# snap-research/GiGL

Hardware: AMD Instinct MI355X
Metric: sampled+aggregated edges/s (higher is better)
Workload: dtype f32

## Files before the change

### gigl_amd/csrc/union.hip

```cpp
#include "common.h"

#include <mutex>

#include <cstdlib>

static hipError_t lds_opt_in(int device, int site, const void* fn, int bytes, const void* fn2 = nullptr, int bytes2 = 0) {
  static std::mutex mu;
  static uint32_t done[256] = {0};
  std::lock_guard<std::mutex> lk(mu);
  const uint32_t bit = 1u << site;
  uint32_t& d = done[device & 255];
  if (d & bit) return hipSuccess;
  hipError_t e = hipFuncSetAttribute(fn, hipFuncAttributeMaxDynamicSharedMemorySize, bytes);
  if (e == hipSuccess && fn2) e = hipFuncSetAttribute(fn2, hipFuncAttributeMaxDynamicSharedMemorySize, bytes2);
  if (e == hipSuccess) d |= bit;
  return e;
}

static bool lg_big_cap_wide() {
  static const bool wide = [] {
    const char* e = getenv("GIGL_LG_BIG_CAP");
    return !(e && atoi(e) > 0 && atoi(e) <= 4096);
  }();
  return wide;
// ... 1508 lines not shown
    hipLaunchKernelGGL(lg2_insert_kernel, grid(T_in), dim3(TB), 0, st, a, g);
    hipLaunchKernelGGL(lg2_extras_kernel, grid(S0), dim3(TB), 0, st, a, g);
  }
  {
    gigl_prof_scope ps(ctx, GIGL_K_UNION_NODES);
    hipLaunchKernelGGL(lg2_count_kernel, dim3((unsigned)n_tiles), dim3(256), 0, st, a, g, tile_counts, n_tiles,
                       ticket_count);
    hipLaunchKernelGGL(lg2_assign_kernel, dim3((unsigned)n_tiles), dim3(256), 0, st, a, g, tile_counts, n_tiles,
                       out->nodes, out->meta, out->rowptr, out->rowend, cursor, edge_counters + 32, sort_rows,
                       sort_count, tiny_rows, tiny_count);
  }
  {
    gigl_prof_scope ps(ctx, GIGL_K_UNION_EDGE_SORT);
    hipLaunchKernelGGL(lg2_fill_kernel, grid(T_in), dim3(TB), 0, st, a, g, out->rowend, out->col, out->root_local,
                       out->rowptr);
  }
  {
    gigl_prof_scope ps(ctx, GIGL_K_UNION_CSR);
    {
      int64_t tb = (T_in / 16 + 255) / 256;
      if (tb > 1024) tb = 1024;
      if (tb < 16) tb = 16;
      hipLaunchKernelGGL(lg2_row_sort_tiny_kernel, dim3((unsigned)tb), dim3(256), 0, st, tiny_rows, tiny_count,
                         out->rowptr, out->rowend, out->col, edge_counters);
    }
    int64_t blocks = (T_in / 8 + 3) / 4;
    if (blocks > 256 * 16) blocks = 256 * 16;
    if (blocks < 64) blocks = 64;
    hipLaunchKernelGGL(lg2_row_sort_kernel, dim3((unsigned)blocks), dim3(256), 0, st, sort_rows, sort_count,
                       out->rowptr, out->rowend, out->col, big_rows, big_count, edge_counters);
    if (lg_big_cap_wide()) {
      GIGL_HIP_CHECK(ctx, lds_opt_in(ctx->device, 0, (const void*)lg2_row_sort_big_kernel<BIG_ROW_CAP>, 2 * BIG_ROW_CAP * (int)sizeof(int32_t)));
      hipLaunchKernelGGL(lg2_row_sort_big_kernel<BIG_ROW_CAP>, dim3(8), dim3(1024), 2 * BIG_ROW_CAP * sizeof(int32_t), st,
                       out->rowptr, out->rowend, out->col, big_rows, big_count, out->meta + GIGL_META_OVERFLOW,
                       edge_counters, ticket_big, out->meta);
    } else
    hipLaunchKernelGGL(lg2_row_sort_big_kernel<LG_BIG_CAP>, dim3(8), dim3(1024), 2 * LG_BIG_CAP * sizeof(int32_t), st,
                       out->rowptr, out->rowend, out->col, big_rows, big_count, out->meta + GIGL_META_OVERFLOW,
                       edge_counters, ticket_big, out->meta);
  }
  GIGL_HIP_CHECK(ctx, hipGetLastError());
  return GIGL_OK;
}


constexpr int LG3_CODE_BITS = 20;
constexpr uint32_t LG3_CODE_MASK = (1u << LG3_CODE_BITS) - 1u;
constexpr uint32_t LG3_EMPTY = 0xFFFFFFFFu;
constexpr int32_t LG3_XTAG = 1 << 30;
constexpr int LG3_MAX_PARTS = 16;
constexpr int LG3_NT_DEFAULT = 512;
constexpr int LG3_CAP_DEFAULT = 16384;

struct Lg3Args {
  const uint32_t* roots;
  const uint32_t* nbr0;
  const uint32_t* nbr1;
  const int32_t* cnt0;
  const int32_t* cnt1;
  int32_t b, f0, f1;
  int64_t S0;
  int32_t gr;
  int32_t S0g;
  int32_t Tg;
  int32_t n_groups;
  int32_t P;
  uint32_t cmask;
  uint32_t rmask;
  int32_t rs_shift;
  int32_t bl_shift;
  int32_t* fpw;
  int32_t* fpx;
  int32_t* lid_in;
  int32_t* rowcnt;
  int32_t alias_base;
  int32_t whole_rows;
  int32_t* overflow;
};

__device__ __forceinline__ uint32_t lg3_part(uint32_t h32, int P) { return (uint32_t)(((uint64_t)h32 * (uint32_t)P) >> 32); }

__device__ __forceinline__ int64_t lg3_gpos(const Lg3Args& a, int32_t grp, uint32_t code) {
  return code < (uint32_t)a.gr ? (int64_t)grp * a.gr + code : (int64_t)a.b + (int64_t)grp * a.S0g + (code - a.gr);
}

__device__ __forceinline__ void lg3_locate(const Lg3Args& a, int64_t t, int32_t& grp, uint32_t& code) {
  if (t < a.b) {
    grp = a.n_groups == 1 ? 0 : (int32_t)((uint32_t)t / (uint32_t)a.gr);
    code = (uint32_t)(t - (int64_t)grp * a.gr);
  } else {
    const uint32_t p = (uint32_t)(t - a.b);
    grp = a.n_groups == 1 ? 0 : (int32_t)(p / (uint32_t)a.S0g);
    code = (uint32_t)a.gr + (p - (uint32_t)grp * (uint32_t)a.S0g);
  }
}

__device__ __forceinline__ bool lg3_insert(unsigned long long* table, const Lg3Args& a, uint32_t id, uint32_t h32,
                                           uint32_t code) {
  const unsigned long long mine1 = ((unsigned long long)id << 32) | ((unsigned long long)code << 1) | 1ull;
  uint32_t s = h32 & a.cmask;
  for (uint32_t probes = 0; probes <= a.cmask; ++probes) {
    unsigned long long w = table[s];
    if (w == ~0ull) {
      w = atomicCAS(&table[s], ~0ull, mine1);
      if (w == ~0ull) return true;
    }
    if ((uint32_t)(w >> 32) == id) {
      atomicMin(&table[s], mine1 & ~1ull);
      atomicAnd(&table[s], ~1ull);
      return true;
    }
    s = (s + 1) & a.cmask;
  }
  return false;
}

__device__ __forceinline__ uint32_t lg3_lookup(const unsigned long long* table, const Lg3Args& a, uint32_t id,
                                               uint32_t h32) {
  uint32_t s = h32 & a.cmask;
  for (uint32_t probes = 0; probes <= a.cmask; ++probes) {
    const unsigned long long w = table[s];
    if (w == ~0ull) return LG3_EMPTY;
    if ((uint32_t)(w >> 32) == id) return (uint32_t)w;
    s = (s + 1) & a.cmask;
  }
  return LG3_EMPTY;
}

__device__ __forceinline__ bool lg3_rset_has(const uint32_t* rset, const Lg3Args& a, uint32_t id, uint32_t h32) {
  uint32_t s = (h32 * 0x9E3779B1u) >> a.rs_shift;
  for (;;) {
    const uint32_t k = rset[s];
    if (k == id) return true;
    if (k == GIGL_INVALID) return false;
    s = (s + 1) & a.rmask;
  }
}

__device__ __forceinline__ bool lg3_contributes(const Lg3Args& a, uint32_t first_code, uint32_t my_code, int c) {
  if (c >= a.f1 || !a.whole_rows) return true;
  return first_code == my_code || first_code < (uint32_t)a.gr;
}

__device__ __forceinline__ bool lg3_row_is_segment(const Lg3Args& a, uint32_t code, int c) {
  return a.alias_base >= 0 && a.whole_rows && c < a.f1 && code >= (uint32_t)a.gr;
}

constexpr int LG3_TC = 5;

template <int NT>
__global__ __launch_bounds__(NT) void lg3_dedup_kernel(Lg3Args a, int32_t* tile_counts, int32_t n_tiles,
                                                         int32_t* ticket, int32_t* sort_count, int32_t* tiny_count) {
  extern __shared__ unsigned long long lg3_lds[];
  unsigned long long* table = lg3_lds;
  uint32_t* rset = reinterpret_cast<uint32_t*>(table + (a.cmask + 1u));
  uint32_t* bloom = rset + (a.rmask + 1u);
  int32_t* tcnt = reinterpret_cast<int32_t*>(bloom + ((a.rmask + 1u) >> 2));
  __shared__ int32_t s_last;
  __shared__ int32_t s_w[NT / 64][LG3_TC];
  const int tid = threadIdx.x, lane = tid & 63, wv = tid >> 6;
  uint32_t vid = blockIdx.x;
  if ((gridDim.x & 7u) == 0) vid = (blockIdx.x >> 3) + (blockIdx.x & 7u) * (gridDim.x >> 3);
  const int32_t grp = (int32_t)(vid / (uint32_t)a.P);
  const int q = (int)(vid % (uint32_t)a.P);
  const int64_t r0 = (int64_t)grp * a.gr, p0 = (int64_t)grp * a.S0g;
  const int32_t tile_lo_r = (int32_t)(r0 >> 10), nt_r = (int32_t)((r0 + a.gr - 1) >> 10) - tile_lo_r + 1;
  const int32_t tile_lo_h = (int32_t)((a.b + p0) >> 10), nt_h = (int32_t)((a.b + p0 + a.S0g - 1) >> 10) - tile_lo_h + 1;
  for (uint32_t i = tid; i <= a.cmask; i += NT) table[i] = ~0ull;
  for (uint32_t i = tid; i <= a.rmask; i += NT) rset[i] = GIGL_INVALID;
  for (uint32_t i = tid; i < ((a.rmask + 1u) >> 2); i += NT) bloom[i] = 0u;
  for (int i = tid; i < LG3_TC * (nt_r + nt_h); i += NT) tcnt[i] = 0;
  __syncthreads();
  int32_t over = 0;
  for (int32_t tl = tid; tl < a.gr; tl += NT) {
    const uint32_t id = a.roots[r0 + tl];
    if (id == GIGL_INVALID) continue;
    const uint32_t h = hash_u32(id);
    uint32_t s = (h * 0x9E3779B1u) >> a.rs_shift;
    for (;;) {
      const uint32_t prev = atomicCAS(&rset[s], GIGL_INVALID, id);
      if (prev == GIGL_INVALID || prev == id) break;
      s = (s + 1) & a.rmask;
    }
    const uint32_t bi = (h * 0x85EBCA6Bu) >> a.bl_shift;
    atomicOr(&bloom[bi >> 5], 1u << (bi & 31));
    if ((int)lg3_part(h, a.P) == q && !lg3_insert(table, a, id, h, (uint32_t)tl)) ++over;
  }
  __syncthreads();
  constexpr int PF = 8;
  unsigned long long rootmask = 0;
  for (int32_t base = 0, it0 = 0; base < a.S0g; base += PF * NT, it0 += PF) {
    uint32_t ids[PF], hh[PF], sl[PF], bw[PF];
    uint32_t pend = 0, valid = 0;
#pragma unroll
    for (int u = 0; u < PF; ++u) {
      const int32_t pl = base + u * NT + tid;
      ids[u] = pl < a.S0g ? a.nbr0[p0 + pl] : GIGL_INVALID;
    }
#pragma unroll
    for (int u = 0; u < PF; ++u) {
      hh[u] = hash_u32(ids[u]);
      sl[u] = hh[u] & a.cmask;
      const uint32_t bi = (hh[u] * 0x85EBCA6Bu) >> a.bl_shift;
      bw[u] = (bloom[bi >> 5] >> (bi & 31)) & 1u;
      if (ids[u] != GIGL_INVALID) {
        valid |= 1u << u;
        if ((int)lg3_part(hh[u], a.P) == q) pend |= 1u << u;
      }
    }
    for (uint32_t rounds = 0; pend; ++rounds) {
      if (rounds > a.cmask) {
        over += __popc(pend);
        break;
      }
      unsigned long long old[PF];
#pragma unroll
      for (int u = 0; u < PF; ++u)
        if (pend >> u & 1u)
          old[u] = atomicCAS(&table[sl[u]], ~0ull,
                             ((unsigned long long)ids[u] << 32) | ((unsigned long long)(uint32_t)(a.gr + base + u * NT + tid) << 1) | 1ull);
#pragma unroll
      for (int u = 0; u < PF; ++u) {
        if (!(pend >> u & 1u)) continue;
        if (old[u] == ~0ull) {
          pend &= ~(1u << u);
        } else if ((uint32_t)(old[u] >> 32) == ids[u]) {
          atomicMin(&table[sl[u]], ((unsigned long long)ids[u] << 32) | ((unsigned long long)(uint32_t)(a.gr + base + u * NT + tid) << 1));
          atomicAnd(&table[sl[u]], ~1ull);
          pend &= ~(1u << u);
        } else {
          sl[u] = (sl[u] + 1) & a.cmask;
        }
      }
    }
#pragma unroll
    for (int u = 0; u < PF; ++u) {
      if (!((valid >> u & 1u) && bw[u])) continue;
      if (!lg3_rset_has(rset, a, ids[u], hh[u])) continue;
      rootmask |= 1ull << (it0 + u);
      const int32_t pl = base + u * NT + tid;
      const int c = a.cnt1[p0 + pl];
      const uint32_t* kids = a.nbr1 + (p0 + pl) * a.f1;
      for (int j = 0; j < c; ++j) {
        const uint32_t cid = kids[j];
        const uint32_t ch = hash_u32(cid);
        if ((int)lg3_part(ch, a.P) == q && !lg3_insert(table, a, cid, ch, (uint32_t)(a.Tg + pl * a.f1 + j))) ++over;
      }
    }
  }
  if (over) atomicAdd(a.overflow, over);
  __syncthreads();
  for (int32_t tl = tid; tl < a.gr; tl += NT) {
    const uint32_t id = a.roots[r0 + tl];
    if (id == GIGL_INVALID) {
      if (q == 0) a.fpw[r0 + tl] = -1;
      continue;
    }
    const uint32_t h = hash_u32(id);
    if ((int)lg3_part(h, a.P) != q) continue;
    const uint32_t w = lg3_lookup(table, a, id, h);
    if (w == LG3_EMPTY) {
      a.fpw[r0 + tl] = -1;
      continue;
    }
    const uint32_t code = (w >> 1) & LG3_CODE_MASK;
    a.fpw[r0 + tl] = (int32_t)(code | ((w & 1u) ? 0u : 0x80000000u));
    if (code == (uint32_t)tl) atomicAdd(&tcnt[LG3_TC * (int)(((r0 + tl) >> 10) - tile_lo_r) + 0], 1);
    const int c0 = a.cnt0[r0 + tl];
    if (c0 > 0) atomicAdd(&a.rowcnt[r0 + code], c0);
  }
  for (int32_t base = 0, it0 = 0; base < a.S0g; base += PF * NT, it0 += PF) {
    uint32_t ids[PF], sl[PF], lw[PF];
    int32_t cc[PF];
    uint32_t pend = 0;
#pragma unroll
    for (int u = 0; u < PF; ++u) {
      const int32_t pl = base + u * NT + tid;
      ids[u] = pl < a.S0g ? a.nbr0[p0 + pl] : GIGL_INVALID;
      cc[u] = pl < a.S0g ? a.cnt1[p0 + pl] : 0;
    }
#pragma unroll
    for (int u = 0; u < PF; ++u) {
      const uint32_t h = hash_u32(ids[u]);
      sl[u] = h & a.cmask;
      lw[u] = LG3_EMPTY;
      if (ids[u] != GIGL_INVALID && (int)lg3_part(h, a.P) == q) pend |= 1u << u;
    }
    const uint32_t mine = pend;
    for (uint32_t rounds = 0; pend && rounds <= a.cmask; ++rounds) {
      unsigned long long wv8[PF];
#pragma unroll
      for (int u = 0; u < PF; ++u)
        if (pend >> u & 1u) wv8[u] = table[sl[u]];
#pragma unroll
      for (int u = 0; u < PF; ++u) {
        if (!(pend >> u & 1u)) continue;
        if (wv8[u] == ~0ull) {
          pend &= ~(1u << u);
        } else if ((uint32_t)(wv8[u] >> 32) == ids[u]) {
          lw[u] = (uint32_t)wv8[u];
          pend &= ~(1u << u);
        } else {
          sl[u] = (sl[u] + 1) & a.cmask;
        }
      }
    }
#pragma unroll
    for (int u = 0; u < PF; ++u) {
      const int32_t pl = base + u * NT + tid;
      const uint32_t id = ids[u];
      const int c = cc[u];
      const bool in = pl < a.S0g;
      const int32_t my_tile = (int32_t)((a.b + p0 + pl) >> 10) - tile_lo_h;
      bool first = false;
      if (in && id == GIGL_INVALID) {
        if (q == 0) a.fpw[a.b + p0 + pl] = -1;
      } else if (in && (mine >> u & 1u)) {
        const uint32_t mycode = (uint32_t)(a.gr + pl);
        const uint32_t w = lw[u];
        if (w == LG3_EMPTY) {
          a.fpw[a.b + p0 + pl] = -1;
        } else {
          const uint32_t code = (w >> 1) & LG3_CODE_MASK;
          const bool multi = !(w & 1u);
          a.fpw[a.b + p0 + pl] = (int32_t)(code | (multi ? 0x80000000u : 0u));
          first = code == mycode;
          if ((multi || a.alias_base < 0) && c > 0 && !lg3_row_is_segment(a, code, c) && lg3_contributes(a, code, mycode, c))
            atomicAdd(&a.rowcnt[lg3_gpos(a, grp, code)], c);
        }
      }
      {
        const int32_t tile0 = __builtin_amdgcn_readfirstlane(my_tile);
        const unsigned long long f0m = __ballot(first && my_tile == tile0), f1m = __ballot(first && my_tile != tile0);
        if (lane == 0) {
          if (f0m) atomicAdd(&tcnt[LG3_TC * (nt_r + tile0) + 1], (int32_t)__popcll(f0m));
          if (f1m) atomicAdd(&tcnt[LG3_TC * (nt_r + tile0 + 1) + 1], (int32_t)__popcll(f1m));
        }
      }
      if (rootmask >> (it0 + u) & 1ull) {
        const uint32_t* kids = a.nbr1 + (p0 + pl) * a.f1;
        for (int j = 0; j < c; ++j) {
          const uint32_t cid = kids[j];
          const uint32_t ch = hash_u32(cid);
          if ((int)lg3_part(ch, a.P) != q) continue;
          const uint32_t xcode = (uint32_t)(a.Tg + pl * a.f1 + j);
          const uint32_t w = lg3_lookup(table, a, cid, ch);
          int32_t out = -1;
          if (w != LG3_EMPTY) {
            const uint32_t code = (w >> 1) & LG3_CODE_MASK;
            out = (int32_t)(code | ((w & 1u) ? 0u : 0x80000000u));
            if (code == xcode) atomicAdd(&tcnt[LG3_TC * (nt_r + my_tile) + 1], 1);
          }
          a.fpx[(p0 + pl) * a.f1 + j] = out;
        }
      }
    }
  }
  __syncthreads();
  for (int32_t tl = tid; tl < a.gr; tl += NT) {
    const uint32_t id = a.roots[r0 + tl];
    if (id == GIGL_INVALID || (int)lg3_part(hash_u32(id), a.P) != q) continue;
    const int32_t w = a.fpw[r0 + tl];
    if (w == -1 || ((uint32_t)w & 0x7FFFFFFFu) != (uint32_t)tl) continue;
    const int32_t len = __hip_atomic_load(&a.rowcnt[r0 + tl], __ATOMIC_RELAXED, __HIP_MEMORY_SCOPE_AGENT);
    int32_t* tc = &tcnt[LG3_TC * (int)(((r0 + tl) >> 10) - tile_lo_r)];
    if (len) atomicAdd(&tc[2], len);
    if (len >= 2 && w < 0) atomicAdd(&tc[len > TINY_ROW ? 3 : 4], 1);
  }
  for (int32_t base = 0; base < a.S0g; base += PF * NT) {
    uint32_t ids[PF];
    int32_t cc[PF], ww[PF], len[PF];
#pragma unroll
    for (int u = 0; u < PF; ++u) {
      const int32_t pl = base + u * NT + tid;
      ids[u] = pl < a.S0g ? a.nbr0[p0 + pl] : GIGL_INVALID;
      cc[u] = pl < a.S0g ? a.cnt1[p0 + pl] : 0;
      ww[u] = pl < a.S0g ? a.fpw[a.b + p0 + pl] : -1;
    }
#pragma unroll
    for (int u = 0; u < PF; ++u) {
      const int32_t pl = base + u * NT + tid;
      len[u] = -1;
      if (ids[u] == GIGL_INVALID || ww[u] == -1 || (int)lg3_part(hash_u32(ids[u]), a.P) != q) continue;
      const uint32_t mycode = (uint32_t)(a.gr + pl);
      if (((uint32_t)ww[u] & 0x7FFFFFFFu) != mycode) continue;
      const bool multi = ww[u] < 0;
      if (a.alias_base >= 0 && (!multi || lg3_row_is_segment(a, mycode, cc[u]))) continue;
      len[u] = __hip_atomic_load(&a.rowcnt[a.b + p0 + pl], __ATOMIC_RELAXED, __HIP_MEMORY_SCOPE_AGENT);
    }
#pragma unroll
    for (int u = 0; u < PF; ++u) {
      const int32_t pl = base + u * NT + tid;
      const int32_t my_tile = (int32_t)((a.b + p0 + pl) >> 10) - tile_lo_h;
      const int32_t tile0 = __builtin_amdgcn_readfirstlane(my_tile);
      const bool have = len[u] > 0, sorted = len[u] >= 2 && ww[u] < 0;
      if (!__ballot(have)) continue;
      const bool t0 = my_tile == tile0;
      const unsigned long long q0 = __ballot(sorted && len[u] > TINY_ROW && t0), q1 = __ballot(sorted && len[u] > TINY_ROW && !t0);
      const unsigned long long s0 = __ballot(sorted && len[u] <= TINY_ROW && t0), s1 = __ballot(sorted && len[u] <= TINY_ROW && !t0);
      const int32_t n0 = __builtin_amdgcn_readlane(gigl_wave_incl_scan(have && t0 ? len[u] : 0), 63);
      const int32_t n1 = __builtin_amdgcn_readlane(gigl_wave_incl_scan(have && !t0 ? len[u] : 0), 63);
      if (lane == 0) {
        int32_t* tc = &tcnt[LG3_TC * (nt_r + tile0)];
        if (n0) atomicAdd(&tc[2], n0);
        if (q0) atomicAdd(&tc[3], (int32_t)__popcll(q0));
        if (s0) atomicAdd(&tc[4], (int32_t)__popcll(s0));
        if (n1) atomicAdd(&tc[LG3_TC + 2], n1);
        if (q1) atomicAdd(&tc[LG3_TC + 3], (int32_t)__popcll(q1));
        if (s1) atomicAdd(&tc[LG3_TC + 4], (int32_t)__popcll(s1));
      }
    }
  }
  __syncthreads();
  for (int i = tid; i < LG3_TC * (nt_r + nt_h); i += NT) {
    const int32_t v = tcnt[i];
    if (v) {
      const int k = i / LG3_TC;
      const int32_t tile = k < nt_r ? tile_lo_r + k : tile_lo_h + (k - nt_r);
      atomicAdd(&tile_counts[tile * LG3_TC + (i - k * LG3_TC)], v);
    }
  }
  __syncthreads();
  if (tid == 0) {
    __threadfence();
    s_last = atomicAdd(ticket, 1) == (int32_t)gridDim.x - 1 ? 1 : 0;
  }
  __syncthreads();
  if (!s_last) return;
  __builtin_amdgcn_fence(__ATOMIC_ACQUIRE, "agent");
  int32_t run[LG3_TC];
#pragma unroll
  for (int c = 0; c < LG3_TC; ++c) run[c] = 0;
  for (int32_t t0 = 0; t0 < n_tiles; t0 += NT) {
    const int32_t i = t0 + tid;
    int32_t v[LG3_TC], inc[LG3_TC];
#pragma unroll
    for (int c = 0; c < LG3_TC; ++c) {
      v[c] = i < n_tiles ? __hip_atomic_load(&tile_counts[i * LG3_TC + c], __ATOMIC_RELAXED, __HIP_MEMORY_SCOPE_AGENT) : 0;
      inc[c] = gigl_wave_incl_scan(v[c]);
    }
    if (lane == 63) {
#pragma unroll
      for (int c = 0; c < LG3_TC; ++c) s_w[wv][c] = inc[c];
    }
    __syncthreads();
#pragma unroll
    for (int c = 0; c < LG3_TC; ++c) {
      int32_t before = 0, tot = 0;
      for (int k = 0; k < NT / 64; ++k) {
        const int32_t x = s_w[k][c];
        if (k < wv) before += x;
        tot += x;
      }
      if (i < n_tiles) tile_counts[i * LG3_TC + c] = run[c] + before + inc[c] - v[c];
      run[c] += tot;
    }
    __syncthreads();
  }
  if (tid == 0) {
#pragma unroll
    for (int c = 0; c < LG3_TC; ++c) tile_counts[n_tiles * LG3_TC + c] = run[c];
    *sort_count = run[3];
    *tiny_count = run[4];
  }
}

__global__ __launch_bounds__(256) void lg3_init_kernel(int32_t* rowcnt, int64_t n_rowcnt, int32_t* zeros, int64_t zero_words,
                                                       int32_t* meta) {
  const int64_t stride = (int64_t)gridDim.x * blockDim.x;
  const int64_t t0 = (int64_t)blockIdx.x * blockDim.x + threadIdx.x;
  for (int64_t i = t0; i < n_rowcnt; i += stride) rowcnt[i] = 0;
  for (int64_t i = t0; i < zero_words; i += stride) zeros[i] = 0;
  if (t0 < GIGL_META_LEN) meta[t0] = 0;
}

__device__ __forceinline__ void lg3_firsts(const Lg3Args& a, int64_t t, int32_t& w_out, int32_t& grp, uint32_t& mycode,
                                           int& c0, int& c1, uint32_t& own_first, unsigned long long& xmask,
                                           bool& root_parent) {
  c0 = c1 = 0;
  own_first = 0;
  xmask = 0;
  root_parent = false;
  w_out = -1;
  grp = 0;
  mycode = 0;
  if (t >= a.b + a.S0) return;
  const int32_t w = a.fpw[t];
  w_out = w;
  if (w == -1) return;
  lg3_locate(a, t, grp, mycode);
  const uint32_t code = (uint32_t)w & 0x7FFFFFFFu;
  if (code == mycode) {
    own_first = 1;
    if (t < a.b) c0 = 1; else c1 = 1;
  }
  if (t >= a.b && code < (uint32_t)a.gr) {
    root_parent = true;
    const int64_t p = t - a.b;
    const int c = a.cnt1[p];
    const uint32_t xbase = (uint32_t)a.Tg + (mycode - (uint32_t)a.gr) * (uint32_t)a.f1;
    for (int j = 0; j < c; ++j) {
      const int32_t x = a.fpx[p * a.f1 + j];
      if (x != -1 && ((uint32_t)x & 0x7FFFFFFFu) == xbase + j) {
        xmask |= 1ull << j;
        ++c1;
      }
    }
  }
}

__global__ __launch_bounds__(256) void lg3_assign_kernel(Lg3Args a, const int32_t* tile_counts, int32_t n_tiles,
                                                         uint32_t* nodes, int32_t* meta, int32_t* rowptr, int32_t* rowend,
                                                         int32_t* tile_edges, int32_t* sort_rows, int32_t* tiny_rows) {
  __shared__ int32_t s_w[TILE / 64 + 1][5];
  __shared__ int32_t s_alias[4];
  const int tid = threadIdx.x, lane = tid & 63, w = tid >> 6;
  const int32_t* tcb = tile_counts + (int64_t)blockIdx.x * LG3_TC;
  const int32_t before0 = tcb[0], before1 = tcb[1];
  const int32_t s_row_base = tcb[2], s_q_base = tcb[3], s_t_base = tcb[4];
  const int32_t total0 = tile_counts[n_tiles * LG3_TC + 0], total1 = tile_counts[n_tiles * LG3_TC + 1];
  const int64_t base = (int64_t)blockIdx.x * TILE;
  const unsigned long long below = (1ull << lane) - 1ull;
  int32_t fw[TILE / 256];
  int k0[TILE / 256], k1[TILE / 256];
  uint32_t own[TILE / 256];
  unsigned long long xm[TILE / 256];
  int32_t own_len[TILE / 256];
  int32_t x0[TILE / 256], x1[TILE / 256], xn[TILE / 256], xq[TILE / 256], xt[TILE / 256];
#pragma unroll
  for (int r = 0; r < TILE / 256; ++r) {
    const int64_t t = base + r * 256 + tid;
    int32_t grp;
    uint32_t mycode;
    bool rp;
    lg3_firsts(a, t, fw[r], grp, mycode, k0[r], k1[r], own[r], xm[r], rp);
    int32_t nd = 0, nq = 0, nt = 0;
    own_len[r] = 0;
    if (own[r]) {
      const bool multi = fw[r] < 0;
      const bool alias = a.alias_base >= 0 && t >= a.b && (!multi || lg3_row_is_segment(a, mycode, a.cnt1[t - a.b]));
      own_len[r] = alias ? -1 : a.rowcnt[t];
      if (!alias) {
        nd += own_len[r];
        const bool sort_it = own_len[r] >= 2 && multi;
        nq = sort_it && own_len[r] > TINY_ROW ? 1 : 0;
        nt = sort_it && own_len[r] <= TINY_ROW ? 1 : 0;
      }
    }
    const unsigned long long m0 = __ballot(k0[r] != 0), mq = __ballot(nq != 0), mt = __ballot(nt != 0);
    const int32_t i1 = gigl_wave_incl_scan(k1[r]), in = gigl_wave_incl_scan(nd);
    x0[r] = (int32_t)__popcll(m0 & below);
    x1[r] = i1 - k1[r];
    xn[r] = in - nd;
    xq[r] = (int32_t)__popcll(mq & below);
    xt[r] = (int32_t)__popcll(mt & below);
    if (lane == 63) {
      s_w[r * 4 + w][0] = (int32_t)__popcll(m0);
      s_w[r * 4 + w][1] = i1;
      s_w[r * 4 + w][2] = in;
      s_w[r * 4 + w][3] = (int32_t)__popcll(mq);
      s_w[r * 4 + w][4] = (int32_t)__popcll(mt);
    }
  }
  __syncthreads();
  if (w == 0) {
    int32_t v[5], e[5];
#pragma unroll
    for (int c = 0; c < 5; ++c) {
      v[c] = lane < TILE / 64 ? s_w[lane][c] : 0;
      e[c] = gigl_wave_incl_scan(v[c]) - v[c];
    }
#pragma unroll
    for (int c = 0; c < 5; ++c)
      if (lane <= TILE / 64) s_w[lane][c] = e[c];
  }
  __syncthreads();
  int32_t alias_c = 0;
#pragma unroll
  for (int r = 0; r < TILE / 256; ++r) {
    if (!(k0[r] | k1[r])) continue;
    const int32_t* pre = s_w[r * 4 + w];
    int32_t p0 = before0 + x0[r] + pre[0], p1 = total0 + before1 + x1[r] + pre[1], pn = s_row_base + xn[r] + pre[2],
            pq = s_q_base + xq[r] + pre[3], pt = s_t_base + xt[r] + pre[4];
    const int64_t t = base + r * 256 + tid;
    if (own[r]) {
      const bool multi = fw[r] < 0;
      const int32_t id = k0[r] ? p0 : p1++;
      a.lid_in[t] = id;
      nodes[id] = t < a.b ? a.roots[t] : a.nbr0[t - a.b];
      if (own_len[r] < 0) {
        const int64_t p = t - a.b;
        const int32_t c = a.cnt1[p];
        rowptr[id] = a.alias_base + (int32_t)(p * a.f1);
        rowend[id] = a.alias_base + (int32_t)(p * a.f1) + c;
        alias_c += c;
      } else {
        const bool sorted_later = own_len[r] >= 2 && multi;
        rowptr[id] = pn;
        rowend[id] = sorted_later || own_len[r] < 2 ? pn : pn + own_len[r];
        pn += own_len[r];
        if (sorted_later && own_len[r] > TINY_ROW) sort_rows[pq] = id;
        else if (sorted_later) tiny_rows[pt] = id;
        else alias_c += own_len[r];
      }
    }
    if (xm[r]) {
      const int64_t p = t - a.b;
      for (int j = 0; j < a.f1; ++j) {
        if (!(xm[r] >> j & 1ull)) continue;
        const int32_t id = p1++;
        a.fpx[p * a.f1 + j] = id | LG3_XTAG;
        nodes[id] = a.nbr1[p * a.f1 + j];
        rowptr[id] = pn;
        rowend[id] = pn;
      }
    }
  }
  {
    for (int off = 32; off > 0; off >>= 1) alias_c += __shfl_xor(alias_c, off, 64);
    if (lane == 0) s_alias[w] = alias_c;
    __syncthreads();
    if (tid == 0) tile_edges[blockIdx.x] = s_alias[0] + s_alias[1] + s_alias[2] + s_alias[3];
  }
  if (blockIdx.x == 0 && tid == 0) {
    meta[GIGL_META_LEVEL0] = total0;
    meta[GIGL_META_LEVEL0 + 1] = total0 + total1;
    meta[GIGL_META_LEVEL0 + 2] = total0 + total1;
    meta[GIGL_META_N_NODES] = total0 + total1;
    rowptr[total0 + total1] = 0;
    rowend[total0 + total1] = 0;
  }
}

__global__ __launch_bounds__(256) void lg3_fill_kernel(Lg3Args a, int32_t* rowend, int32_t* col, int32_t* root_local,
                                                       const int32_t* rowptr) {
  const int64_t t = (int64_t)blockIdx.x * blockDim.x + threadIdx.x;
  const int lane = threadIdx.x & 63;
  const bool in = t < a.b + a.S0;
  const int32_t w = in ? a.fpw[t] : -1;
  const bool valid = w != -1;
  int32_t grp = 0;
  uint32_t mycode = 0;
  if (in) lg3_locate(a, t, grp, mycode);
  const uint32_t code = (uint32_t)w & 0x7FFFFFFFu;
  const bool multi = valid && w < 0;
  const int32_t lid = valid ? a.lid_in[lg3_gpos(a, grp, code)] : -1;
  if (in && t < a.b) root_local[t] = lid;
  const bool edge = in && t >= a.b && valid;
  bool e_ok = false;
  int32_t dl = 0;
  if (edge) {
    const int64_t rt = (int64_t)((uint32_t)(t - a.b) / (uint32_t)a.f0);
    const int32_t wr = a.fpw[rt];
    if (wr != -1) {
      e_ok = true;
      const int64_t rpos = (int64_t)grp * a.gr + ((uint32_t)wr & 0x7FFFFFFFu);
      dl = a.lid_in[rpos];
      if (wr >= 0 && a.rowcnt[rpos] >= 2) {
        col[rowptr[dl] + (int32_t)((uint32_t)(t - a.b) % (uint32_t)a.f0)] = lid;
        e_ok = false;
      }
    }
  }
  int total, rank, first;
  seg_rank(e_ok ? (uint32_t)dl : (0x80000000u | (uint32_t)lane), e_ok, lane, total, rank, first);
  int32_t basep = 0;
  if (e_ok && rank == 0) basep = atomicAdd(&rowend[dl], total);
  basep = __shfl(basep, first, 64);
  if (e_ok) col[basep + rank] = lid;
  if (edge && (multi || a.alias_base < 0)) {
    const int64_t p = t - a.b;
    const int c = a.cnt1[p];
    if (c > 0 && !lg3_row_is_segment(a, code, c) && lg3_contributes(a, code, mycode, c)) {
      const int32_t at = atomicAdd(&rowend[lid], c);
      const bool local = code < (uint32_t)a.gr;
      const int64_t xg = (int64_t)grp * a.S0g * a.f1;
      for (int j = 0; j < c; ++j) {
        int32_t v = (int32_t)a.nbr1[p * a.f1 + j];
        if (local) {
          int32_t x = a.fpx[p * a.f1 + j];
          v = 0;
          if (x != -1) {
            if (!(x & LG3_XTAG)) {
              const uint32_t c2 = (uint32_t)x & 0x7FFFFFFFu;
              x = c2 < (uint32_t)a.Tg ? a.lid_in[lg3_gpos(a, grp, c2)] | LG3_XTAG : a.fpx[xg + (c2 - a.Tg)];
            }
            v = x & (LG3_XTAG - 1);
          }
        }
        col[at + j] = v;
      }
    }
  }
}

int32_t union_build_lg3(gigl_ctx* ctx, const uint32_t* roots, const gigl_tree* tree, int32_t group_roots,
                        gigl_union* out, bool multiset_rows, bool* taken) {
  *taken = false;
  const int b = tree->b;
  const int f0 = tree->fanouts[0], f1 = tree->fanouts[1];
  const int64_t S0 = (int64_t)b * f0, S1 = S0 * f1, T_in = b + S0;
  const int64_t n_groups = b / group_roots;
  const int64_t gr = group_roots, Tg = gr * (1 + f0), S1g = gr * f0 * f1;
  static const int lg3_nt_env = [] {
    const char* e = getenv("GIGL_LG3_NT");
    const int v = e ? atoi(e) : 0;
    return v == 512 || v == 1024 ? v : 0;
  }();
  int lg3_nt = lg3_nt_env ? lg3_nt_env : (gr * f0 <= 64 * (int64_t)LG3_NT_DEFAULT ? LG3_NT_DEFAULT : 1024);
  if (Tg + S1g >= (int64_t)LG3_CODE_MASK || f1 > 64 || b + S0 + S1 >= ((int64_t)1 << 31) || gr * f0 > 64 * (int64_t)lg3_nt) return GIGL_OK;
  static const int64_t cap_max = [] {
    const char* e = getenv("GIGL_LG3_CAP");
    const int64_t v = e ? atoll(e) : 0;
    return v >= 1024 && v <= 16384 && (v & (v - 1)) == 0 ? v : (int64_t)LG3_CAP_DEFAULT;
  }();
  int64_t cap = 1024;
  while (cap < 2 * Tg && cap < cap_max) cap <<= 1;
  const int64_t P = (2 * Tg + cap - 1) / cap;
  if (P > LG3_MAX_PARTS) return GIGL_OK;
  if (!lg3_nt_env && n_groups * P < 256) lg3_nt = 1024;
  static const int64_t min_wgs = getenv("GIGL_LG3_MIN_WGS") ? atoll(getenv("GIGL_LG3_MIN_WGS")) : 32;
  if (n_groups * P < min_wgs) return GIGL_OK;
  int64_t rs = 64;
  int rs_log2 = 6;
  while (rs < 2 * gr) {
    rs <<= 1;
    ++rs_log2;
  }
  const int64_t n_tcnt = LG3_TC * ((gr >> 10) + 2 + ((gr * f0) >> 10) + 2);
  const size_t lds_bytes = (size_t)cap * 8 + (size_t)(rs + rs / 4 + n_tcnt) * 4;
  if (lds_bytes > 150 * 1024) return GIGL_OK;
  *taken = true;
  hipStream_t st = ctx->stream;
  const int32_t n_tiles = (int32_t)((T_in + TILE - 1) / TILE);
  constexpr int EC_STRIDE = 32;
  const int64_t zero_words = 64 + 32 * EC_STRIDE + (int64_t)(n_tiles + 1) * LG3_TC;
  int64_t need = 0;
  auto add = [&](int64_t bytes) { need += gigl_align_up(bytes, 256); };
  add(zero_words * 4);
  add((int64_t)n_tiles * 4);
  add(T_in * 4);
  add(T_in * 4);
  add(T_in * 4);
  add(S1 * 4);
  add(T_in * 4);
  add(T_in * 4);
  add(T_in * 4);
  int32_t rc = gigl_arena_reset(ctx, need + 4096);
  if (rc != GIGL_OK) return rc;
  int32_t* zeros = (int32_t*)gigl_arena_alloc(ctx, zero_words * 4);
  int32_t* tile_edges = (int32_t*)gigl_arena_alloc(ctx, (int64_t)n_tiles * 4);
  Lg3Args a{};
  a.fpw = (int32_t*)gigl_arena_alloc(ctx, T_in * 4);
  a.lid_in = (int32_t*)gigl_arena_alloc(ctx, T_in * 4);
  a.rowcnt = (int32_t*)gigl_arena_alloc(ctx, T_in * 4);
  a.fpx = (int32_t*)gigl_arena_alloc(ctx, S1 * 4);
  int32_t* big_rows = (int32_t*)gigl_arena_alloc(ctx, T_in * 4);
  int32_t* sort_rows = (int32_t*)gigl_arena_alloc(ctx, T_in * 4);
  int32_t* tiny_rows = (int32_t*)gigl_arena_alloc(ctx, T_in * 4);
  if (!zeros || !tile_edges || !a.fpw || !a.lid_in || !a.rowcnt || !a.fpx || !big_rows || !sort_rows || !tiny_rows)
    return gigl_fail(ctx, GIGL_E_OOM, "arena exhausted");
  a.roots = roots;
  a.nbr0 = tree->nbr[0];
  a.nbr1 = tree->nbr[1];
  a.cnt0 = tree->cnt[0];
  a.cnt1 = tree->cnt[1];
  a.b = b;
  a.f0 = f0;
  a.f1 = f1;
  a.S0 = S0;
  a.gr = (int32_t)gr;
  a.S0g = (int32_t)(gr * f0);
  a.Tg = (int32_t)Tg;
  a.n_groups = (int32_t)n_groups;
  a.P = (int32_t)P;
  a.cmask = (uint32_t)(cap - 1);
  a.rmask = (uint32_t)(rs - 1);
  a.rs_shift = 32 - rs_log2;
  a.bl_shift = 32 - (rs_log2 + 3);
  a.whole_rows = multiset_rows ? 0 : 1;
  a.overflow = out->meta + GIGL_META_OVERFLOW;
  a.alias_base = -1;
  if (tree->nbr[1] == (const uint32_t*)(out->col + out->cap_edges) && out->cap_edges + S1 < ((int64_t)1 << 31))
    a.alias_base = (int32_t)out->cap_edges;
  int32_t* ticket_count = zeros + 1;
  int32_t* ticket_big = zeros + 2;
  int32_t* big_count = zeros + 3;
  int32_t* sort_count = zeros + 4;
  int32_t* tiny_count = zeros + 5;
  int32_t* edge_counters = zeros + 64;
  int32_t* tile_counts = zeros + 64 + 32 * EC_STRIDE;
  const int TB = 256;
  auto grid = [&](int64_t n) { return dim3((unsigned)((n + TB - 1) / TB)); };
  GIGL_HIP_CHECK(ctx, lds_opt_in(ctx->device, 1, (const void*)lg3_dedup_kernel<1024>, 150 * 1024));
  GIGL_HIP_CHECK(ctx, lds_opt_in(ctx->device, 3, (const void*)lg3_dedup_kernel<512>, 150 * 1024));
  {
    gigl_prof_scope ps(ctx, GIGL_K_UNION_INSERT);
    hipLaunchKernelGGL(lg3_init_kernel, dim3(256), dim3(256), 0, st, a.rowcnt, T_in, zeros, zero_words, out->meta);
    if (lg3_nt == 512)
      hipLaunchKernelGGL(lg3_dedup_kernel<512>, dim3((unsigned)(n_groups * P)), dim3(512), lds_bytes, st, a, tile_counts,
                         n_tiles, ticket_count, sort_count, tiny_count);
    else
      hipLaunchKernelGGL(lg3_dedup_kernel<1024>, dim3((unsigned)(n_groups * P)), dim3(1024), lds_bytes, st, a, tile_counts,
                         n_tiles, ticket_count, sort_count, tiny_count);
  }
  {
    gigl_prof_scope ps(ctx, GIGL_K_UNION_NODES);
    hipLaunchKernelGGL(lg3_assign_kernel, dim3((unsigned)n_tiles), dim3(256), 0, st, a, tile_counts, n_tiles, out->nodes,
                       out->meta, out->rowptr, out->rowend, tile_edges, sort_rows, tiny_rows);
  }
  {
    gigl_prof_scope ps(ctx, GIGL_K_UNION_EDGE_SORT);
    hipLaunchKernelGGL(lg3_fill_kernel, grid(T_in), dim3(TB), 0, st, a, out->rowend, out->col, out->root_local, out->rowptr);
  }
  {
    gigl_prof_scope ps(ctx, GIGL_K_UNION_CSR);
    {
      static const int64_t tiny_div = getenv("GIGL_LG3_TINY_DIV") ? atoll(getenv("GIGL_LG3_TINY_DIV")) : 4;
      int64_t tb = (T_in / (tiny_div > 0 ? tiny_div : 4) + 255) / 256;
      if (tb > 4096) tb = 4096;
      if (tb < 16) tb = 16;
      hipLaunchKernelGGL(lg2_row_sort_tiny_kernel, dim3((unsigned)tb), dim3(256), 0, st, tiny_rows, tiny_count,
                         out->rowptr, out->rowend, out->col, edge_counters, EC_STRIDE);
    }
    int64_t blocks = (T_in / 8 + 3) / 4;
    if (blocks > 256 * 16) blocks = 256 * 16;
    if (blocks < 64) blocks = 64;
    hipLaunchKernelGGL(lg2_row_sort_kernel, dim3((unsigned)blocks), dim3(256), 0, st, sort_rows, sort_count, out->rowptr,
                       out->rowend, out->col, big_rows, big_count, edge_counters, EC_STRIDE);
    if (lg_big_cap_wide()) {
      GIGL_HIP_CHECK(ctx, lds_opt_in(ctx->device, 4, (const void*)lg2_row_sort_big_kernel<BIG_ROW_CAP>, 2 * BIG_ROW_CAP * (int)sizeof(int32_t)));
      hipLaunchKernelGGL(lg2_row_sort_big_kernel<BIG_ROW_CAP>, dim3(8), dim3(1024), 2 * BIG_ROW_CAP * sizeof(int32_t), st, out->rowptr,
                       out->rowend, out->col, big_rows, big_count, out->meta + GIGL_META_OVERFLOW, edge_counters,
                       ticket_big, out->meta, EC_STRIDE, (const int32_t*)tile_edges, n_tiles);
    } else
    hipLaunchKernelGGL(lg2_row_sort_big_kernel<LG_BIG_CAP>, dim3(8), dim3(1024), 2 * LG_BIG_CAP * sizeof(int32_t), st, out->rowptr,
                       out->rowend, out->col, big_rows, big_count, out->meta + GIGL_META_OVERFLOW, edge_counters,
                       ticket_big, out->meta, EC_STRIDE, (const int32_t*)tile_edges, n_tiles);
  }
  GIGL_HIP_CHECK(ctx, hipGetLastError());
  return GIGL_OK;
}

}

extern "C" {

int32_t gigl_union_capacity(int32_t b, const int32_t* fanouts, int32_t hops, int64_t* cap_nodes,
                            int64_t* cap_edges) {
  if (!fanouts || hops < 1 || hops > GIGL_MAX_HOPS || b < 0) return GIGL_E_INVALID_ARG;
  int64_t parents = b, edges = 0;
  for (int k = 0; k < hops; ++k) {
    parents *= fanouts[k];
    edges += parents;
  }
  if (cap_nodes) *cap_nodes = edges + b;
  if (cap_edges) *cap_edges = edges;
  return GIGL_OK;
}

int32_t gigl_union_build(gigl_ctx* ctx, const uint32_t* roots, const gigl_tree* tree,
                         gigl_union* out) {
  if (!ctx) return GIGL_E_INVALID_ARG;
  GIGL_REQUIRE(ctx, tree, "null argument");
  return gigl_union_build_groups(ctx, roots, tree, tree->b, out);
}

int32_t gigl_union_build_groups(gigl_ctx* ctx, const uint32_t* roots, const gigl_tree* tree,
                                int32_t group_roots, gigl_union* out) {
  return gigl_union_build_impl(ctx, roots, tree, group_roots, out, 0);
}

}

int32_t gigl_union_build_impl(gigl_ctx* ctx, const uint32_t* roots, const gigl_tree* tree, int32_t group_roots,
                              gigl_union* out, int32_t leaf_global) {
  if (!ctx) return GIGL_E_INVALID_ARG;
  GIGL_REQUIRE(ctx, tree && out && (roots || tree->b == 0), "null argument");
  GIGL_REQUIRE(ctx, !leaf_global || tree->hops <= 2, "leaf-global union needs hops <= 2");
  GIGL_REQUIRE(ctx, out->meta && out->nodes && out->rowptr && out->rowend && out->col && out->root_local,
               "union output buffers are null");
  const int hops = tree->hops, b = tree->b;
  GIGL_REQUIRE(ctx, hops >= 1 && hops <= GIGL_MAX_HOPS && b >= 0, "bad tree");
  int64_t cap_nodes, cap_edges;
  gigl_union_capacity(b, tree->fanouts, hops, &cap_nodes, &cap_edges);
  GIGL_REQUIRE(ctx, out->cap_nodes >= cap_nodes && out->cap_edges >= cap_edges,
               "union buffers too small: need %lld nodes / %lld edges", (long long)cap_nodes,
               (long long)cap_edges);
  GIGL_HIP_CHECK(ctx, hipSetDevice(ctx->device));
  hipStream_t st = ctx->stream;
  if (b == 0) {
    GIGL_HIP_CHECK(ctx, hipMemsetAsync(out->meta, 0, GIGL_META_LEN * sizeof(int32_t), st));
    GIGL_HIP_CHECK(ctx, hipMemsetAsync(out->rowptr, 0, sizeof(int32_t), st));
    GIGL_HIP_CHECK(ctx, hipMemsetAsync(out->rowend, 0, sizeof(int32_t), st));
    return GIGL_OK;
  }
  if (leaf_global && hops == 2 && !getenv("GIGL_UNION_GENERIC")) {
    GIGL_REQUIRE(ctx, group_roots >= 1 && b % group_roots == 0, "group_roots=%d does not divide b=%d", group_roots, b);
    static const bool keep_lg2 = getenv("GIGL_UNION_LG2") != nullptr;
    if (!keep_lg2) {
      bool taken = false;
      const int32_t rc3 = union_build_lg3(ctx, roots, tree, group_roots, out, (leaf_global & 2) != 0, &taken);
      if (rc3 != GIGL_OK || taken) return rc3;
    }
    return union_build_lg2(ctx, roots, tree, group_roots, out, (leaf_global & 2) != 0);
  }

  UnionArgs a{};
  a.roots = roots;
  a.b = b;
  a.hops = hops;
  a.leaf_global = leaf_global ? 1 : 0;
  int64_t T = b, parents = b;
  for (int k = 0; k < hops; ++k) {
    a.nbr[k] = tree->nbr[k];
    a.fan[k] = tree->fanouts[k];
    a.off[k] = T;
    parents *= tree->fanouts[k];
    T += parents;
  }
  a.off[hops] = T;
  a.T = T;
  GIGL_REQUIRE(ctx, T < (int64_t)1 << 31, "batch too large: %lld stream positions", (long long)T);
  int64_t n_groups = 1;
  if (group_roots != b) {
    GIGL_REQUIRE(ctx, group_roots >= 1 && b % group_roots == 0, "group_roots=%d does not divide b=%d", group_roots, b);
    n_groups = b / group_roots;
    a.grouped = 1;
    a.group_roots = (uint32_t)group_roots;
    int64_t per_group = group_roots;
    for (int k = 0; k < hops; ++k) {
      per_group *= tree->fanouts[k];
      a.gdiv[k] = (uint32_t)per_group;
    }
  }
  const int64_t E = T - b;
  const int64_t max_rows = a.off[hops - 1];
  uint64_t cap = 1024, ecap = 1024;
  int64_t inner = b / n_groups, width = b / n_groups;
  for (int k = 0; k + 1 < hops; ++k) {
    width *= tree->fanouts[k];
    inner += width;
  }
  const uint64_t want = a.leaf_global ? (uint64_t)inner * 4 : (uint64_t)(T / n_groups) * 3;
  while (cap * 2 < want) cap <<= 1;
  while (ecap * 2 < (uint64_t)(E / n_groups) * 3) ecap <<= 1;
  a.mask = (uint32_t)(cap - 1);
  const int64_t n_slots = (int64_t)cap * n_groups, n_ekeys = (int64_t)ecap * n_groups;
  GIGL_REQUIRE(ctx, n_slots < (int64_t)1 << 31, "batch too large: %lld table slots", (long long)n_slots);
  const int32_t n_tiles = (int32_t)((T + TILE - 1) / TILE);

// ... 79 lines not shown
```

Before: 10.92 billion.

## Compact dedup loops to filled neighbor slots via LDS rank bitmap

The dedup kernel now scans per-root neighbor counts to build an LDS bitmap plus per-run offsets. The three passes over hop-0 neighbor slots then iterate only over filled slots instead of all S0g padded slots, which removes wasted loads and hash work when fanout is not saturated. fpw initialization to -1 moves into the init kernel, and the tile-count ballots become a loop that handles any number of tiles per wave. In exchange it uses more LDS, which can push configurations past the 150KB limit and onto the fallback path, adds a block-wide scan with syncs, adds indirection per slot, and halves the prefetch depth for 1024-thread blocks.

```diff
diff --git a/gigl_amd/csrc/union.hip b/gigl_amd/csrc/union.hip
--- a/gigl_amd/csrc/union.hip
+++ b/gigl_amd/csrc/union.hip
@@ -1684,10 +1684,14 @@
 __global__ __launch_bounds__(NT) void lg3_dedup_kernel(Lg3Args a, int32_t* tile_counts, int32_t n_tiles,
                                                          int32_t* ticket, int32_t* sort_count, int32_t* tiny_count) {
   extern __shared__ unsigned long long lg3_lds[];
+  const uint32_t nm = ((uint32_t)a.S0g + 63u) >> 6;
   unsigned long long* table = lg3_lds;
-  uint32_t* rset = reinterpret_cast<uint32_t*>(table + (a.cmask + 1u));
+  unsigned long long* fbits = table + (a.cmask + 1u);
+  uint32_t* rset = reinterpret_cast<uint32_t*>(fbits + nm);
   uint32_t* bloom = rset + (a.rmask + 1u);
-  int32_t* tcnt = reinterpret_cast<int32_t*>(bloom + ((a.rmask + 1u) >> 2));
+  int32_t* frank = reinterpret_cast<int32_t*>(bloom + ((a.rmask + 1u) >> 2));
+  int32_t* fdelta = frank + nm;
+  int32_t* tcnt = fdelta + a.gr;
   __shared__ int32_t s_last;
   __shared__ int32_t s_w[NT / 64][LG3_TC];
   const int tid = threadIdx.x, lane = tid & 63, wv = tid >> 6;
@@ -1702,7 +1706,44 @@
   for (uint32_t i = tid; i <= a.rmask; i += NT) rset[i] = GIGL_INVALID;
   for (uint32_t i = tid; i < ((a.rmask + 1u) >> 2); i += NT) bloom[i] = 0u;
   for (int i = tid; i < LG3_TC * (nt_r + nt_h); i += NT) tcnt[i] = 0;
+  for (uint32_t i = tid; i < nm; i += NT) fbits[i] = 0ull;
+  if (tid == 0 && nm) frank[0] = 0;
   __syncthreads();
+  int32_t n_fill = 0, n_runs = 0;
+  for (int32_t rb = 0; rb < a.gr; rb += NT) {
+    const int32_t r = rb + tid;
+    int32_t c = r < a.gr ? a.cnt0[r0 + r] : 0;
+    c = c < 0 ? 0 : (c > a.f0 ? a.f0 : c);
+    const int32_t ic = gigl_wave_incl_scan(c), ir = gigl_wave_incl_scan(c > 0 ? 1 : 0);
+    if (lane == 63) {
+      s_w[wv][0] = ic;
+      s_w[wv][1] = ir;
+    }
+    __syncthreads();
+    int32_t bc = 0, br = 0, tc = 0, tr = 0;
+    for (int k = 0; k < NT / 64; ++k) {
+      if (k < wv) {
+        bc += s_w[k][0];
+        br += s_w[k][1];
+      }
+      tc += s_w[k][0];
+      tr += s_w[k][1];
+    }
+    if (c > 0) {
+      const int32_t start = n_fill + bc + ic - c, k = n_runs + br + ir - 1;
+      fdelta[k] = r * a.f0 - start;
+      atomicOr(&fbits[start >> 6], 1ull << (start & 63));
+      for (int32_t m = (start + 64) >> 6; m < (int32_t)nm && (m << 6) <= start + c; ++m) frank[m] = k + 1;
+    }
+    n_fill += tc;
+    n_runs += tr;
+    __syncthreads();
+  }
+  auto slot_of = [&](int32_t i) -> int32_t {
+    const uint32_t m = (uint32_t)i >> 6;
+    const int32_t k = frank[m] + (int32_t)__popcll(fbits[m] & (~0ull >> (63 - lane))) - 1;
+    return i + fdelta[k];
+  };
   int32_t over = 0;
   for (int32_t tl = tid; tl < a.gr; tl += NT) {
     const uint32_t id = a.roots[r0 + tl];
@@ -1719,15 +1760,17 @@
     if ((int)lg3_part(h, a.P) == q && !lg3_insert(table, a, id, h, (uint32_t)tl)) ++over;
   }
   __syncthreads();
-  constexpr int PF = 8;
+  constexpr int PF = NT >= 1024 ? 4 : 8;
   unsigned long long rootmask = 0;
-  for (int32_t base = 0, it0 = 0; base < a.S0g; base += PF * NT, it0 += PF) {
+  for (int32_t base = 0, it0 = 0; base < n_fill; base += PF * NT, it0 += PF) {
+    int32_t pls[PF];
     uint32_t ids[PF], hh[PF], sl[PF], bw[PF];
     uint32_t pend = 0, valid = 0;
 #pragma unroll
     for (int u = 0; u < PF; ++u) {
-      const int32_t pl = base + u * NT + tid;
-      ids[u] = pl < a.S0g ? a.nbr0[p0 + pl] : GIGL_INVALID;
+      const int32_t i = base + u * NT + tid;
+      pls[u] = i < n_fill ? slot_of(i) : -1;
+      ids[u] = pls[u] >= 0 ? a.nbr0[p0 + pls[u]] : GIGL_INVALID;
     }
 #pragma unroll
     for (int u = 0; u < PF; ++u) {
@@ -1750,14 +1793,14 @@
       for (int u = 0; u < PF; ++u)
         if (pend >> u & 1u)
           old[u] = atomicCAS(&table[sl[u]], ~0ull,
-                             ((unsigned long long)ids[u] << 32) | ((unsigned long long)(uint32_t)(a.gr + base + u * NT + tid) << 1) | 1ull);
+                             ((unsigned long long)ids[u] << 32) | ((unsigned long long)(uint32_t)(a.gr + pls[u]) << 1) | 1ull);
 #pragma unroll
       for (int u = 0; u < PF; ++u) {
         if (!(pend >> u & 1u)) continue;
         if (old[u] == ~0ull) {
           pend &= ~(1u << u);
         } else if ((uint32_t)(old[u] >> 32) == ids[u]) {
-          atomicMin(&table[sl[u]], ((unsigned long long)ids[u] << 32) | ((unsigned long long)(uint32_t)(a.gr + base + u * NT + tid) << 1));
+          atomicMin(&table[sl[u]], ((unsigned long long)ids[u] << 32) | ((unsigned long long)(uint32_t)(a.gr + pls[u]) << 1));
           atomicAnd(&table[sl[u]], ~1ull);
           pend &= ~(1u << u);
         } else {
@@ -1770,7 +1813,7 @@
       if (!((valid >> u & 1u) && bw[u])) continue;
       if (!lg3_rset_has(rset, a, ids[u], hh[u])) continue;
       rootmask |= 1ull << (it0 + u);
-      const int32_t pl = base + u * NT + tid;
+      const int32_t pl = pls[u];
       const int c = a.cnt1[p0 + pl];
       const uint32_t* kids = a.nbr1 + (p0 + pl) * a.f1;
       for (int j = 0; j < c; ++j) {
@@ -1784,32 +1827,27 @@
   __syncthreads();
   for (int32_t tl = tid; tl < a.gr; tl += NT) {
     const uint32_t id = a.roots[r0 + tl];
-    if (id == GIGL_INVALID) {
-      if (q == 0) a.fpw[r0 + tl] = -1;
-      continue;
-    }
+    if (id == GIGL_INVALID) continue;
     const uint32_t h = hash_u32(id);
     if ((int)lg3_part(h, a.P) != q) continue;
     const uint32_t w = lg3_lookup(table, a, id, h);
-    if (w == LG3_EMPTY) {
-      a.fpw[r0 + tl] = -1;
-      continue;
-    }
+    if (w == LG3_EMPTY) continue;
     const uint32_t code = (w >> 1) & LG3_CODE_MASK;
     a.fpw[r0 + tl] = (int32_t)(code | ((w & 1u) ? 0u : 0x80000000u));
     if (code == (uint32_t)tl) atomicAdd(&tcnt[LG3_TC * (int)(((r0 + tl) >> 10) - tile_lo_r) + 0], 1);
     const int c0 = a.cnt0[r0 + tl];
     if (c0 > 0) atomicAdd(&a.rowcnt[r0 + code], c0);
   }
-  for (int32_t base = 0, it0 = 0; base < a.S0g; base += PF * NT, it0 += PF) {
+  for (int32_t base = 0, it0 = 0; base < n_fill; base += PF * NT, it0 += PF) {
     uint32_t ids[PF], sl[PF], lw[PF];
-    int32_t cc[PF];
+    int32_t pcs[PF];
     uint32_t pend = 0;
 #pragma unroll
     for (int u = 0; u < PF; ++u) {
-      const int32_t pl = base + u * NT + tid;
-      ids[u] = pl < a.S0g ? a.nbr0[p0 + pl] : GIGL_INVALID;
-      cc[u] = pl < a.S0g ? a.cnt1[p0 + pl] : 0;
+      const int32_t i = base + u * NT + tid;
+      const int32_t pl = i < n_fill ? slot_of(i) : -1;
+      ids[u] = pl >= 0 ? a.nbr0[p0 + pl] : GIGL_INVALID;
+      pcs[u] = pl >= 0 ? (pl << 8) | a.cnt1[p0 + pl] : -256;
     }
 #pragma unroll
     for (int u = 0; u < PF; ++u) {
@@ -1839,15 +1877,11 @@
     }
 #pragma unroll
     for (int u = 0; u < PF; ++u) {
-      const int32_t pl = base + u * NT + tid;
-      const uint32_t id = ids[u];
-      const int c = cc[u];
-      const bool in = pl < a.S0g;
+      const int32_t pl = pcs[u] >> 8;
+      const int c = pcs[u] & 255;
       const int32_t my_tile = (int32_t)((a.b + p0 + pl) >> 10) - tile_lo_h;
       bool first = false;
-      if (in && id == GIGL_INVALID) {
-        if (q == 0) a.fpw[a.b + p0 + pl] = -1;
-      } else if (in && (mine >> u & 1u)) {
+      if (mine >> u & 1u) {
         const uint32_t mycode = (uint32_t)(a.gr + pl);
         const uint32_t w = lw[u];
         if (w == LG3_EMPTY) {
@@ -1861,13 +1895,11 @@
             atomicAdd(&a.rowcnt[lg3_gpos(a, grp, code)], c);
         }
       }
-      {
-        const int32_t tile0 = __builtin_amdgcn_readfirstlane(my_tile);
-        const unsigned long long f0m = __ballot(first && my_tile == tile0), f1m = __ballot(first && my_tile != tile0);
-        if (lane == 0) {
-          if (f0m) atomicAdd(&tcnt[LG3_TC * (nt_r + tile0) + 1], (int32_t)__popcll(f0m));
-          if (f1m) atomicAdd(&tcnt[LG3_TC * (nt_r + tile0 + 1) + 1], (int32_t)__popcll(f1m));
-        }
+      for (unsigned long long todo = __ballot(first); todo;) {
+        const int32_t tile0 = __builtin_amdgcn_readlane(my_tile, (int)__builtin_ctzll(todo));
+        const unsigned long long fm = __ballot(first && my_tile == tile0);
+        if (lane == 0) atomicAdd(&tcnt[LG3_TC * (nt_r + tile0) + 1], (int32_t)__popcll(fm));
+        todo &= ~fm;
       }
       if (rootmask >> (it0 + u) & 1ull) {
         const uint32_t* kids = a.nbr1 + (p0 + pl) * a.f1;
@@ -1899,19 +1931,20 @@
     if (len) atomicAdd(&tc[2], len);
     if (len >= 2 && w < 0) atomicAdd(&tc[len > TINY_ROW ? 3 : 4], 1);
   }
-  for (int32_t base = 0; base < a.S0g; base += PF * NT) {
+  for (int32_t base = 0; base < n_fill; base += PF * NT) {
     uint32_t ids[PF];
-    int32_t cc[PF], ww[PF], len[PF];
+    int32_t pls[PF], cc[PF], ww[PF], len[PF];
 #pragma unroll
     for (int u = 0; u < PF; ++u) {
-      const int32_t pl = base + u * NT + tid;
-      ids[u] = pl < a.S0g ? a.nbr0[p0 + pl] : GIGL_INVALID;
-      cc[u] = pl < a.S0g ? a.cnt1[p0 + pl] : 0;
-      ww[u] = pl < a.S0g ? a.fpw[a.b + p0 + pl] : -1;
+      const int32_t i = base + u * NT + tid;
+      pls[u] = i < n_fill ? slot_of(i) : -1;
+      ids[u] = pls[u] >= 0 ? a.nbr0[p0 + pls[u]] : GIGL_INVALID;
+      cc[u] = pls[u] >= 0 ? a.cnt1[p0 + pls[u]] : 0;
+      ww[u] = pls[u] >= 0 ? a.fpw[a.b + p0 + pls[u]] : -1;
     }
 #pragma unroll
     for (int u = 0; u < PF; ++u) {
-      const int32_t pl = base + u * NT + tid;
+      const int32_t pl = pls[u];
       len[u] = -1;
       if (ids[u] == GIGL_INVALID || ww[u] == -1 || (int)lg3_part(hash_u32(ids[u]), a.P) != q) continue;
       const uint32_t mycode = (uint32_t)(a.gr + pl);
@@ -1922,24 +1955,21 @@
     }
 #pragma unroll
     for (int u = 0; u < PF; ++u) {
-      const int32_t pl = base + u * NT + tid;
-      const int32_t my_tile = (int32_t)((a.b + p0 + pl) >> 10) - tile_lo_h;
-      const int32_t tile0 = __builtin_amdgcn_readfirstlane(my_tile);
+      const int32_t my_tile = (int32_t)((a.b + p0 + pls[u]) >> 10) - tile_lo_h;
       const bool have = len[u] > 0, sorted = len[u] >= 2 && ww[u] < 0;
-      if (!__ballot(have)) continue;
-      const bool t0 = my_tile == tile0;
-      const unsigned long long q0 = __ballot(sorted && len[u] > TINY_ROW && t0), q1 = __ballot(sorted && len[u] > TINY_ROW && !t0);
-      const unsigned long long s0 = __ballot(sorted && len[u] <= TINY_ROW && t0), s1 = __ballot(sorted && len[u] <= TINY_ROW && !t0);
-      const int32_t n0 = __builtin_amdgcn_readlane(gigl_wave_incl_scan(have && t0 ? len[u] : 0), 63);
-      const int32_t n1 = __builtin_amdgcn_readlane(gigl_wave_incl_scan(have && !t0 ? len[u] : 0), 63);
-      if (lane == 0) {
-        int32_t* tc = &tcnt[LG3_TC * (nt_r + tile0)];
-        if (n0) atomicAdd(&tc[2], n0);
-        if (q0) atomicAdd(&tc[3], (int32_t)__popcll(q0));
-        if (s0) atomicAdd(&tc[4], (int32_t)__popcll(s0));
-        if (n1) atomicAdd(&tc[LG3_TC + 2], n1);
-        if (q1) atomicAdd(&tc[LG3_TC + 3], (int32_t)__popcll(q1));
-        if (s1) atomicAdd(&tc[LG3_TC + 4], (int32_t)__popcll(s1));
+      for (unsigned long long todo = __ballot(have); todo;) {
+        const int32_t tile0 = __builtin_amdgcn_readlane(my_tile, (int)__builtin_ctzll(todo));
+        const bool t0 = have && my_tile == tile0;
+        const unsigned long long tm = __ballot(t0);
+        const unsigned long long qm = __ballot(t0 && sorted && len[u] > TINY_ROW), sm = __ballot(t0 && sorted && len[u] <= TINY_ROW);
+        const int32_t n = __builtin_amdgcn_readlane(gigl_wave_incl_scan(t0 ? len[u] : 0), 63);
+        if (lane == 0) {
+          int32_t* tc = &tcnt[LG3_TC * (nt_r + tile0)];
+          atomicAdd(&tc[2], n);
+          if (qm) atomicAdd(&tc[3], (int32_t)__popcll(qm));
+          if (sm) atomicAdd(&tc[4], (int32_t)__popcll(sm));
+        }
+        todo &= ~tm;
       }
     }
   }
@@ -1997,11 +2027,14 @@
   }
 }
 
-__global__ __launch_bounds__(256) void lg3_init_kernel(int32_t* rowcnt, int64_t n_rowcnt, int32_t* zeros, int64_t zero_words,
-                                                       int32_t* meta) {
+__global__ __launch_bounds__(256) void lg3_init_kernel(int32_t* rowcnt, int32_t* fpw, int64_t n_rowcnt, int32_t* zeros,
+                                                       int64_t zero_words, int32_t* meta) {
   const int64_t stride = (int64_t)gridDim.x * blockDim.x;
   const int64_t t0 = (int64_t)blockIdx.x * blockDim.x + threadIdx.x;
-  for (int64_t i = t0; i < n_rowcnt; i += stride) rowcnt[i] = 0;
+  for (int64_t i = t0; i < n_rowcnt; i += stride) {
+    rowcnt[i] = 0;
+    fpw[i] = -1;
+  }
   for (int64_t i = t0; i < zero_words; i += stride) zeros[i] = 0;
   if (t0 < GIGL_META_LEN) meta[t0] = 0;
 }
@@ -2260,7 +2293,8 @@
     ++rs_log2;
   }
   const int64_t n_tcnt = LG3_TC * ((gr >> 10) + 2 + ((gr * f0) >> 10) + 2);
-  const size_t lds_bytes = (size_t)cap * 8 + (size_t)(rs + rs / 4 + n_tcnt) * 4;
+  const int64_t nm = (gr * f0 + 63) / 64;
+  const size_t lds_bytes = (size_t)cap * 8 + (size_t)nm * 8 + (size_t)(rs + rs / 4 + nm + gr + n_tcnt) * 4;
   if (lds_bytes > 150 * 1024) return GIGL_OK;
   *taken = true;
   hipStream_t st = ctx->stream;
@@ -2328,7 +2362,7 @@
   GIGL_HIP_CHECK(ctx, lds_opt_in(ctx->device, 3, (const void*)lg3_dedup_kernel<512>, 150 * 1024));
   {
     gigl_prof_scope ps(ctx, GIGL_K_UNION_INSERT);
-    hipLaunchKernelGGL(lg3_init_kernel, dim3(256), dim3(256), 0, st, a.rowcnt, T_in, zeros, zero_words, out->meta);
+    hipLaunchKernelGGL(lg3_init_kernel, dim3(256), dim3(256), 0, st, a.rowcnt, a.fpw, T_in, zeros, zero_words, out->meta);
     if (lg3_nt == 512)
       hipLaunchKernelGGL(lg3_dedup_kernel<512>, dim3((unsigned)(n_groups * P)), dim3(512), lds_bytes, st, a, tile_counts,
                          n_tiles, ticket_count, sort_count, tiny_count);
```

Result: no change. 11.01 billion (median of 6 runs) (+0.8%).
